# google/nerfactor

Measured on AMD Instinct MI355X. Metric: rays/sec (NeRF coarse+fine render, 64+128 samples/ray), higher is better.
Workload: dtype bf16; 1 GPU; lego_3072-shaped NeRF coarse+fine MLP render, 800x800 rays/view, 64+128 samples (BASELINE.json configs[1]); rays_per_view=640000, n_samples_coarse=64, n_samples_fine=128, kernel_variant=7

## Files before the change

include/nfx.h:

```cpp
#ifndef NFX_H_
#define NFX_H_

#include <stddef.h>
#include <stdint.h>

#ifdef __cplusplus
extern "C" {
#endif

#if defined(__GNUC__)
#define NFX_API __attribute__((visibility("default")))
#else
#define NFX_API
#endif

#define NFX_OK 0
#define NFX_EINVAL (-1)
#define NFX_EALIGN (-2)
#define NFX_EHIP (-3)
#define NFX_ENOSUP (-4)

#define NFX_PREC_BF16 0
#define NFX_PREC_FP32 1
#define NFX_PREC_FP32_NATIVE 2
// ... 236 lines not shown
                             void *dev_workspace, size_t workspace_bytes, void *stream);

NFX_API int nfx_nerf_refine_select(const float *dev_rgbs, const float *dev_z, const float *dev_rayd, int64_t n_rays,
                           int n_samples, float t_min, float a_lo, float a_hi, float sigma_margin, int dilate,
                           int *dev_list, int *dev_count, void *stream);
NFX_API int nfx_nerf_sigma_refine(const float *dev_rayo, const float *dev_rayd, const float *dev_z, int64_t n_rays,
                          int n_samples, const void *dev_geom_blob_fp32, const int *dev_list, const int *dev_count,
                          float *dev_rgbs, void *stream);

NFX_API int nfx_nerf_sigma_refine_last(const float *dev_rayo, const float *dev_rayd, const float *dev_z, int64_t n_rays,
                               int n_samples, const void *dev_geom_blob_fp32, float *dev_rgbs, void *stream);

#define NFX_OCCGRID_MAX_RES 1024
#define NFX_OCCGRID_MAX_PROBES (1ll << 30)
NFX_API int nfx_nerf_sigma_fwd_list(const float *dev_rayo, const float *dev_rayd, const float *dev_z, int64_t n_rays,
                            int n_samples, const void *dev_geom_blob, int prec, const int *dev_list,
                            const int *dev_count, float *dev_sigma, void *stream);
NFX_API size_t nfx_occgrid_workspace_bytes(int64_t n_rays, int n_samples);
NFX_API int nfx_occgrid_select(const float *dev_rayo, const float *dev_rayd, const float *dev_z, int64_t n_rays,
                       int n_samples, const uint32_t *dev_bits, int res, const float *box, const float *bbox,
                       float *dev_sigma, void *dev_workspace, size_t workspace_bytes, void *stream);
NFX_API int nfx_occgrid_bake(const float *dev_probe_sigma, int res, int probes, float margin, int dilate,
                     uint32_t *dev_bits, uint32_t *dev_workspace, void *stream);


NFX_API int nfx_selftest_mfma_bf16(const float *dev_a, const float *dev_b, float *dev_d, void *stream);
NFX_API int nfx_mlp_generic_split_hilo(void *dev_blob, int d_in, int n_layers, const int *widths, const int *skip_input,
                                       int train, void *stream);
NFX_API size_t nfx_mlp_generic_packed_bytes(int d_in, int n_layers, const int *widths, const int *skip_input, int prec);
NFX_API int nfx_mlp_generic_pack(const float *const *kernels, const float *const *biases, int d_in, int n_layers,
                                 const int *widths, const int *skip_input, int prec, void *blob, size_t blob_bytes);
NFX_API int nfx_mlp_generic_fwd(const float *dev_x, int64_t n, int ld_x, int d_in, int n_layers, const int *widths,
                                const int *acts, const int *skip_input, const void *dev_blob, int prec, float *dev_y,
                                int ld_y, int col0, void *stream);
NFX_API size_t nfx_mlp_generic_train_packed_bytes(int d_in, int n_layers, const int *widths, const int *skip_input,
                                                  int prec);
NFX_API int nfx_mlp_generic_pack_train(const float *const *kernels, const float *const *biases, int d_in, int n_layers,
                                       const int *widths, const int *skip_input, int prec, void *blob,
                                       size_t blob_bytes);
NFX_API size_t nfx_mlp_generic_bwd_workspace_bytes(int64_t n, int d_in, int n_layers, const int *widths,
                                                   const int *skip_input, int prec);
NFX_API int nfx_mlp_generic_bwd(const float *dev_x, int64_t n, int ld_x, int d_in, int n_layers, const int *widths,
                                const int *acts, const int *skip_input, const void *dev_train_blob, int prec,
                                const float *dev_dy, int ld_dy, int col0_dy, float *dev_dx, int ld_dx,
                                float *const *dev_dkernels, float *const *dev_dbiases, void *dev_workspace,
                                size_t workspace_bytes, void *stream);
NFX_API int nfx_embed_bwd(const float *dev_v, int64_t n, int n_freqs, int incl_input, const float *dev_d_out, int ld_out,
                          int col0, float *dev_dv, void *stream);
NFX_API int nfx_embed(const float *dev_x, const float *dev_dir, const float *dev_z, int64_t n, int per_ray, int mode,
                      int n_freqs, int incl_input, float *dev_out, int ld_out, int col0, void *stream);

NFX_API int nfx_selftest_tr16(const float *dev_h, const float *dev_z, float *dev_d, int mode, void *stream);
NFX_API int nfx_selftest_sincos(const float *dev_in, int64_t n, int which, float *dev_out, void *stream);

NFX_API int nfx_selftest_wgrad_plan(int n_calls, const int *k_in, const int *n_out, int64_t rows, int *use_lds, int *wide,
                                    int64_t *slab, int *n_slabs);
NFX_API size_t nfx_selftest_wgrad_partial_bytes(int n_calls, const int *k_in, const int *n_out, int64_t rows);
NFX_API int nfx_selftest_wgrad_batch(int n_calls, const void *const *dev_xt, const void *const *dev_zt, const int *k_in,
                                     const int *n_out, float *const *dev_dw, float *const *dev_db, int64_t ld, int64_t rows,
                                     const int32_t *dev_count, void *dev_partial, size_t partial_bytes, void *stream);

#ifdef __cplusplus
}
#endif
#endif
```

nerfactor_amd/_capi.py:

```python
import ctypes
import os

import torch

_HERE = os.path.dirname(os.path.abspath(__file__))
LIB_PATH = os.path.join(_HERE, 'libnfx.so')
if os.environ.get('NFX_LIB_PATH'):
    LIB_PATH = os.environ['NFX_LIB_PATH']

PREC_BF16, PREC_FP32, PREC_FP32_NATIVE = 0, 1, 2
ACT_NONE, ACT_RELU, ACT_SIGMOID, ACT_SOFTPLUS = 0, 1, 2, 3
IN_XYZ, IN_XYZ_LDIR, IN_Z_RUSINK = 0, 1, 2

if not os.path.exists(LIB_PATH):
    raise ImportError(
        "%s not found: build it with `python -m nerfactor_amd.build` (or __graft_entry__.build()); "
        "nerfactor_amd has no fallback path." % LIB_PATH)

lib = ctypes.CDLL(LIB_PATH)

_p = ctypes.c_void_p
_i = ctypes.c_int
_i64 = ctypes.c_int64
_f = ctypes.c_float
# ... 33 lines not shown
    'nfx_merl_query': (_i, [_p, _p, _i64, _p, _p, _p]),
    'nfx_merl_sphere_fwd': (_i, [_p, _p, _i64, _p, _p, _p, _p, _i, _p, _p, _p]),
    'nfx_dir2rusink': (_i, [_p, _p, _i64, _p, _p]),
    'nfx_mlp128_train_packed_bytes': (_sz, [_i]),
    'nfx_mlp128_pack_train_weights': (_i, [_pp, _pp, _i, _i, _i, _p, _sz]),
    'nfx_mlp128_bwd_workspace_bytes': (_sz, [_i, _i64, _i]),
    'nfx_mlp128_bwd': (_i, [_i, _p, _p, _i64, _f, _p, _i, _p, _i, _i, _f, _p, _p, _sz, _pp, _pp, _i, _p]),
    'nfx_mlp128_bwd_heads': (_i, [_i, _p, _p, _i64, _f, _p, _i, _i, _pp, _p, _p, _p, _pp, _p, _sz, _pp, _pp, _i, _p]),
    'nfx_composite_bwd': (_i, [_p, _p, _p, _p, _i64, _i, _i, _p, _p, _p]),
    'nfx_nerf_train_packed_bytes': (_sz, [_i]),
    'nfx_nerf_pack_train_weights': (_i, [_pp, _pp, _i, _p, _sz]),
    'nfx_nerf_bwd_workspace_bytes': (_sz, [_i64, _i]),
    'nfx_nerf_mlp_bwd': (_i, [_p, _p, _p, _i64, _i, _p, _i, _p, _p, _sz, _pp, _pp, _p]),
    'nfx_brdf_train_packed_bytes': (_sz, []),
    'nfx_brdf_pack_train_weights': (_i, [_pp, _pp, _i, _i, _p, _sz]),
    'nfx_brdf_spec_bwd_workspace_bytes': (_sz, [_i, _i64]),
    'nfx_brdf_spec_bwd': (_i, [_p, _p, _p, _p, _i, _p, _i, _p, _i, _i64, _p, _p, _p, _p, _sz, _p]),
    'nfx_brdf_spec_bwd_list_bytes': (_sz, [_i64, _i]),
    'nfx_brdf_spec_bwd_rows': (_i, [_p, _p, _p, _p, _i, _p, _i, _p, _i, _i64, _p, _p, _p, _p, _sz, _p, _sz, _p]),
    'nfx_brdf_rows_fwd': (_i, [_p, _i, _p, _i64, _i, _p, _i, _p, _p]),
    'nfx_brdf_rows_bwd_workspace_bytes': (_sz, [_i, _i64, _i]),
    'nfx_brdf_rows_bwd': (_i, [_p, _i, _p, _i64, _i, _p, _i, _p, _p, _sz, _p, _pp, _pp, _p]),
    'nfx_shade_bwd_workspace_bytes': (_sz, [_i]),
    'nfx_shade_bwd': (_i, [_p, _p, _p, _p, _p, _p, _f, _f, _p, _p, _p, _p, _i64, _i, _i, _p, _p, _p, _p, _p, _p,
                           _p, _p, _sz, _p]),
    'nfx_l2_normalize_rows': (_i, [_p, _p, _i64, _i, _f, _p]),
    'nfx_l2_normalize_rows_bwd': (_i, [_p, _p, _p, _i64, _i, _f, _p]),
    'nfx_light_smoothness': (_i, [_p, _i, _i, _f, _f, _p, _p, _p]),
    'nfx_pair_loss_fwd': (_i, [_p, _i, _p, _f, _i64, _p, _p]),
    'nfx_pair_loss_bwd': (_i, [_p, _i, _p, _f, _i64, _p, _p]),
    'nfx_pack_gather': (_i, [_p, _p, _i64, _p, _p]),
    'nfx_amsgrad_step': (_i, [_p, _p, _p, _p, _p, _i64, _f, _f, _f, _f, _i64, _p]),
    'nfx_amsgrad_step_size': (_f, [_f, _f, _f, _i64]),
    'nfx_amsgrad_step_dev': (_i, [_p, _p, _p, _p, _p, _i64, _p, _f, _f, _f, _p]),
    'nfx_nerf_sigma_fwd': (_i, [_p, _p, _p, _i64, _i, _p, _i, _p, _p]),
    'nfx_lvis_fwd_rows': (_i, [_p, _p, _i64, _f, _p, _i, _p, _i, _p, _sz, _p, _p, _p, _p]),
    'nfx_zero_rows': (_i, [_p, _p, _i64, _i, _p]),
    'nfx_shade_fwd_rows': (_i, [_p, _p, _p, _p, _p, _p, _f, _f, _p, _p, _p, _p, _p, _i64, _i, _i, _i, _p, _p]),
    'nfx_shade_olat_fwd_rows': (_i, [_p, _p, _p, _p, _p, _p, _f, _f, _p, _p, _p, _p, _f, _f, _i64, _i, _i, _p, _p, _p, _p]),
    'nfx_nerf_refine_select': (_i, [_p, _p, _p, _i64, _i, _f, _f, _f, _f, _i, _p, _p, _p]),
    'nfx_nerf_sigma_refine': (_i, [_p, _p, _p, _i64, _i, _p, _p, _p, _p, _p]),
    'nfx_nerf_sigma_refine_last': (_i, [_p, _p, _p, _i64, _i, _p, _p, _p]),
    'nfx_nerf_sigma_fwd_list': (_i, [_p, _p, _p, _i64, _i, _p, _i, _p, _p, _p, _p]),
    'nfx_occgrid_workspace_bytes': (_sz, [_i64, _i]),
    'nfx_occgrid_select': (_i, [_p, _p, _p, _i64, _i, _p, _i, _p, _p, _p, _p, _sz, _p]),
    'nfx_occgrid_bake': (_i, [_p, _i, _i, _f, _i, _p, _p, _p]),
    'nfx_nerf_geom_packed_bytes': (_sz, [_i]),
    'nfx_nerf_pack_geom_weights': (_i, [_pp, _pp, _i, _p, _sz]),
    'nfx_nerf_sigma_grad': (_i, [_p, _p, _p, _i64, _i, _p, _i, _p, _p]),
    'nfx_nerf_sigma_grad_workspace_bytes': (_sz, [_i64, _i]),
    'nfx_nerf_sigma_grad_rows': (_i, [_p, _p, _p, _i64, _i, _p, _i, _p, _p, _sz, _p]),
    'nfx_selftest_mfma_bf16': (_i, [_p, _p, _p, _p]),
    'nfx_selftest_sincos': (_i, [_p, _i64, _i, _p, _p]),
    'nfx_selftest_tr16': (_i, [_p, _p, _p, _i, _p]),
    'nfx_selftest_wgrad_plan': (_i, [_i, _p, _p, _i64, _p, _p, _p, _p]),
    'nfx_selftest_wgrad_partial_bytes': (_sz, [_i, _p, _p, _i64]),
    'nfx_selftest_wgrad_batch': (_i, [_i, _pp, _pp, _p, _p, _pp, _pp, _i64, _i64, _p, _p, _sz, _p]),
    'nfx_mlp_generic_packed_bytes': (_sz, [_i, _i, _p, _p, _i]),
    'nfx_mlp_generic_pack': (_i, [_pp, _pp, _i, _i, _p, _p, _i, _p, _sz]),
    'nfx_mlp_generic_fwd': (_i, [_p, _i64, _i, _i, _i, _p, _p, _p, _p, _i, _p, _i, _i, _p]),
    'nfx_mlp_generic_train_packed_bytes': (_sz, [_i, _i, _p, _p, _i]),
    'nfx_mlp_generic_pack_train': (_i, [_pp, _pp, _i, _i, _p, _p, _i, _p, _sz]),
    'nfx_mlp_generic_bwd_workspace_bytes': (_sz, [_i64, _i, _i, _p, _p, _i]),
    'nfx_mlp_generic_split_hilo': (_i, [_p, _i, _i, _p, _p, _i, _p]),
    'nfx_brdf_rows_geom_fwd': (_i, [_p, _p, _p, _p, _i, _p, _i, _i64, _i, _p, _i, _p, _p]),
    'nfx_brdf_rows_geom_bwd': (_i, [_p, _p, _p, _i, _p, _i, _i64, _i, _p, _i, _p, _p, _p]),
    'nfx_embed_bwd': (_i, [_p, _i64, _i, _i, _p, _i, _i, _p, _p]),
    'nfx_mlp_generic_bwd': (_i, [_p, _i64, _i, _i, _i, _p, _p, _p, _p, _i, _p, _i, _i, _p, _i, _pp, _pp, _p, _sz, _p]),
    'nfx_embed': (_i, [_p, _p, _p, _i64, _i, _i, _i, _i, _p, _i, _i, _p]),
}

for _name, (_res, _args) in SIGNATURES.items():
    _fn = getattr(lib, _name)
    _fn.restype = _res
    _fn.argtypes = _args


class NfxError(RuntimeError):
    """Raised for any non-zero return of the C-ABI; mirrors how the reference surfaces failures as
    Python exceptions (tf.errors.InvalidArgumentError from tf.debugging.*)."""


def last_error():
    buf = ctypes.create_string_buffer(512)
    lib.nfx_last_error(buf, 512)
    return buf.value.decode()


def check(rc, what):
    if rc != 0:
        raise NfxError("%s failed (%d): %s" % (what, rc, last_error()))


OPTION_KEYS = ('nerf_variant', 'nerf_fold', 'nerf_blocks', 'm128_blocks', 'lvis_variant', 'brdf_variant', 'brdf_ct', 'nerf_bwd',
               'nerf_bwd_nw', 'm128_bwd', 'wgrad_lds', 'wgrad_slabs', 'wgrad_rounds', 'wgrad_narrow', 'wgrad_fused', 'lvis_verify', 'lvis_rows', 'brdf_bwd_rows', 'nerf_bwd_rows', 'sigma_grad_rows', 'sigma_variant',
               'sigma_x3_variant')


def set_option(key, value):
    check(lib.nfx_set_option(key.encode(), int(value)), 'nfx_set_option(%s)' % key)


def unset_option(key):
    check(lib.nfx_unset_option(key.encode()), 'nfx_unset_option(%s)' % key)


# ... 32 lines not shown
```

nerfactor_amd/csrc/capi.cpp:

```cpp
#include <hip/hip_runtime.h>
#include <stdarg.h>
#include <stdio.h>
#include <stdlib.h>
#include <string.h>

#include <atomic>
#include <vector>

#include "capi_common.hpp"
#include "nerf_layout.hpp"
#include "nerf_fold_layout.hpp"
#include "pack.hpp"

static thread_local char g_err[512] = "";

int nfx_fail(int code, const char* fmt, ...) {
    va_list ap;
    va_start(ap, fmt);
    vsnprintf(g_err, sizeof(g_err), fmt, ap);
    va_end(ap);
    return code;
}
int nfx_hip_result(int e, const char* what) {
    if (e == 0) return NFX_OK;
// ... 244 lines not shown
int nfx_composite_fwd(const float* rgbs, const float* z, const float* rayd, const float* noise,
                      int64_t n_rays, int n_samples, int white_bg, float* rgb, float* occu, float* depth,
                      float* disp, float* weights, void* stream) {
    REQUIRE(n_rays >= 0 && n_samples >= 1, "nfx_composite_fwd: bad shape");
    if (n_rays == 0) return NFX_OK;
    REQUIRE(rgbs && z && rayd, "nfx_composite_fwd: null input");
    if (!ALIGNED(rgbs, 16)) return nfx_fail(NFX_EALIGN, "nfx_composite_fwd: rgbs must be 16-byte aligned");
    return nfx_hip_result(nfx_launch_composite(rgbs, z, rayd, noise, n_rays, n_samples, white_bg, rgb, occu,
                                               depth, disp, weights, (hipStream_t)stream),
                          "composite_fwd");
}

int nfx_nerf_surface_fwd(const float* sigma, const float* z, const float* rayo, const float* rayd, int64_t n_rays,
                         int n_samples, float occu_thres, int quantize_alpha, float* alpha, float* xyz, float* depth,
                         float* occu, void* stream) {
    REQUIRE(n_rays >= 0 && n_samples >= 1, "nfx_nerf_surface_fwd: bad shape (%lld rays, %d samples)", (long long)n_rays,
            n_samples);
    REQUIRE(occu_thres == occu_thres, "nfx_nerf_surface_fwd: occu_thres is NaN");
    if (n_rays == 0) return NFX_OK;
    REQUIRE(sigma && z && rayo && rayd, "nfx_nerf_surface_fwd: null input");
    REQUIRE(alpha && xyz && depth, "nfx_nerf_surface_fwd: null output (only occu may be NULL)");
    return nfx_hip_result(nfx_launch_surface(sigma, z, rayo, rayd, n_rays, n_samples, occu_thres, quantize_alpha ? 1 : 0, alpha,
                                             xyz, depth, occu, (hipStream_t)stream),
                          "nerf_surface_fwd");
}

int nfx_sample_fine(const float* z, const float* weights, int64_t n_rays, int n_coarse, int n_fine,
                    const float* u, float* z_all, void* stream) {
    REQUIRE(n_rays >= 0, "nfx_sample_fine: n_rays < 0");
    REQUIRE(n_coarse <= 258, "nfx_sample_fine: at most 258 coarse samples (256 pdf bins), got %d", n_coarse);
    REQUIRE(n_coarse >= 3 && n_fine >= 2, "nfx_sample_fine: need n_coarse >= 3 and n_fine >= 2 (got %d, %d)",
            n_coarse, n_fine);
    REQUIRE((size_t)4 * (2 * (n_coarse - 1) + n_coarse + n_fine) * 4 <= 64 * 1024,
            "nfx_sample_fine: n_coarse + n_fine too large for one workgroup's LDS");
    if (n_rays == 0) return NFX_OK;
    REQUIRE(z && weights && z_all, "nfx_sample_fine: null pointer");
    return nfx_hip_result(
            nfx_launch_sample_fine(z, weights, n_rays, n_coarse, n_fine, u, z_all, (hipStream_t)stream),
            "sample_fine");
}

int nfx_selftest_mfma_bf16(const float* a, const float* b, float* d, void* stream) {
    REQUIRE(a && b && d, "nfx_selftest_mfma_bf16: null pointer");
    return nfx_hip_result(nfx_launch_selftest_mfma(a, b, d, (hipStream_t)stream), "selftest_mfma");
}
int nfx_selftest_tr16(const float* h, const float* z, float* d, int mode, void* stream) {
    REQUIRE(d && (mode == 1 || (h && z)), "nfx_selftest_tr16: null pointer");
    return nfx_hip_result(nfx_launch_selftest_tr16(h, z, d, mode, (hipStream_t)stream), "selftest_tr16");
}
int nfx_selftest_sincos(const float* in, int64_t n, int which, float* out, void* stream) {
    REQUIRE(n >= 0 && (n == 0 || (in && out)), "nfx_selftest_sincos: bad arguments");
    return nfx_hip_result(nfx_launch_selftest_sincos(in, n, which, out, (hipStream_t)stream), "selftest_sincos");
}

}
```

nerfactor_amd/csrc/launchers.hpp:

```cpp
#pragma once
#include <hip/hip_runtime.h>
#include <stddef.h>
#include <stdint.h>

#include "../../include/nfx.h"

namespace nfx::generic { struct Args; struct EmbedArgs; struct BwdArgs; struct WgradArgs; }
namespace nfx::rowsgeom { struct Args; }
namespace nfx::geo { struct Points; }

struct nfx_wgrad_call {
    const void* xt;
    const void* zt;
    int k_in, n_out;
    float* dw;
    float* db;
};

extern "C" {
int nfx_option_int(const char* key, int dflt);
int nfx_brdf_train_blob_bytes(void);
int nfx_launch_brdf_spec_bwd(const float* xyz, const float* cam, const float* normal, const float* z, int z_dim, const float* lxyz,
                             int n_lights, const void* blob, long long n, const float* dspec, float* d_z, float* d_normal, void* workspace,
                             int max_blocks, hipStream_t st, void* list_ws);
// ... 48 lines not shown
int nfx_launch_split_hilo(void* frags, long long n_frags, hipStream_t st);
int nfx_launch_embed_bwd(const nfx::generic::EmbedArgs* a, const float* d_out, float* dv, hipStream_t st);
int nfx_launch_embed(const nfx::generic::EmbedArgs* a, hipStream_t st);
size_t nfx_nerf_bwd_list_bytes(long long n_pts);
int nfx_launch_nerf_bwd(const float* rayo, const float* rayd, const float* z, long long n_pts, int n_samples, const void* blob,
                        const float* d_rgbs, void* wsp, long long ld, int max_blocks, hipStream_t st, void* list_ws);
int nfx_launch_nerf_fold(const void* blob, void* out, hipStream_t stream);
int nfx_launch_nerf_sigma_grad(const nfx::geo::Points* pts, const void* blob, float* out, int max_blocks, hipStream_t st);
int nfx_launch_select_density(const float* sigma, long long n_pts, float* out, void* list_ws, hipStream_t st);
int nfx_launch_nerf_sigma_geo(const float* rayo, const float* rayd, const float* z, long long n_pts, int n_samples, const void* blob,
                              float* out, int max_blocks, hipStream_t st);
int nfx_launch_nerf_sigma_grad_x3(const nfx::geo::Points* pts, const void* blob, float* out, int max_blocks, hipStream_t st);
int nfx_launch_nerf_sigma_x3(const nfx::geo::Points* pts, const void* blob, float* out, int max_blocks, hipStream_t st);
int nfx_launch_nerf_mlp_bf16(const float* rayo, const float* rayd, const float* z, long long n_pts, int n_samples, const void* blob,
                             float* out, int variant, int max_blocks, hipStream_t stream);
int nfx_launch_nerf_mlp_bf16_fold(const float* rayo, const float* rayd, const float* z, long long n_pts, int n_samples, const void* blob,
                                  float* out, int variant, int max_blocks, hipStream_t stream);
int nfx_launch_nerf_mlp_bf16_v6(const float* rayo, const float* rayd, const float* z, long long n_pts, int n_samples, const void* blob,
                                float* out, int max_blocks, int dma_mode, hipStream_t stream);
int nfx_launch_nerf_mlp_bf16_v6_fold(const float* rayo, const float* rayd, const float* z, long long n_pts, int n_samples, const void* blob,
                                     float* out, int max_blocks, int dma_mode, hipStream_t stream);
int nfx_launch_nerf_mlp_x3(const float* rayo, const float* rayd, const float* z, long long n_pts, int n_samples, const void* blob,
                           float* out, int max_blocks, hipStream_t stream);
int nfx_launch_nerf_sigma_v6(const float* rayo, const float* rayd, const float* z, long long n_pts, int n_samples, const void* blob,
                             float* out, int max_blocks, hipStream_t stream);
int nfx_launch_nerf_sigma_v6_list(const float* rayo, const float* rayd, const float* z, long long capacity, int n_samples, const void* blob,
                                  float* out, const int* list, const int* count, int max_blocks, hipStream_t stream);
int nfx_launch_nerf_sigma_x3_pipe(const nfx::geo::Points* pts, const void* blob, float* out, int max_blocks, hipStream_t st);
size_t nfx_occgrid_list_bytes(long long n_pts);
int nfx_launch_occgrid_select(const float* rayo, const float* rayd, const float* z, long long n_rays, int n_samples, const uint32_t* bits,
                              int res, const float* box, const float* bbox, float* out, void* ws, hipStream_t st);
int nfx_launch_occgrid_bake(const float* sigma, int res, int probes, float margin, int dilate, uint32_t* bits, uint32_t* ws,
                            hipStream_t st);
int nfx_launch_pack_gather(const float* src, const int* map, long long n_words, void* blob, hipStream_t st);
int nfx_launch_l2_normalize3(const float* in, float* out, long long n, float eps, hipStream_t st);
int nfx_launch_gen_z(float near, float far, int n_samples, long long n_rays, int lin_in_disp, const float* u, float* z, hipStream_t st);
int nfx_launch_composite(const float* rgbs, const float* z, const float* rayd, const float* noise, long long n_rays, int S, int white_bg,
                         float* rgb, float* occu, float* depth, float* disp, float* w, hipStream_t st);
int nfx_launch_surface(const float* sigma, const float* z, const float* rayo, const float* rayd, long long n_rays, int S, float occu_thres,
                       int quantize, float* alpha, float* xyz, float* depth, float* occu, hipStream_t st);
int nfx_launch_refine_select(const float* rgbs, const float* z, const float* rayd, long long n_rays, int S, float t_min, float a_lo,
                             float a_hi, float sigma_margin, int dilate, int* list, int* count, hipStream_t st);
int nfx_launch_sample_fine(const float* z, const float* w, long long n_rays, int nc, int nf, const float* u, float* z_all, hipStream_t st);
int nfx_launch_composite_bwd(const float* rgbs, const float* z, const float* rayd, const float* noise, long long n_rays, int n_samples,
                             int white_bg, const float* d_rgb, float* d_rgbs, hipStream_t st);
int nfx_launch_scatter_rows(const float* src, const int* row_of, long long n_all, int d, float* dst, hipStream_t st);
int nfx_launch_zero_rows(float* dst, const int* row_of, long long n_all, int d, hipStream_t st);
int nfx_launch_nonfinite(const float* x, long long n, int* flag, hipStream_t st);
int nfx_launch_l2_normalize_rows(int bwd, const float* x, const float* dy, float* out, long long n, int d, float eps, hipStream_t st);
int nfx_launch_light_smoothness(const float* light, int H, int W, float tv_w, float achro_w, float* loss, float* grad, hipStream_t st);
int nfx_launch_selftest_tr16(const float* h, const float* z, float* d, int mode, hipStream_t st);
int nfx_launch_selftest_mfma(const float* a, const float* b, float* d, hipStream_t st);
int nfx_launch_selftest_sincos(const float* in, long long n, int which, float* out, hipStream_t st);
size_t nfx_shade_olat_lds_bytes(int n_lights);
int nfx_launch_shade(const float* xyz, const float* cam, const float* normal, const float* albedo, const float* rough, const float* spec,
                     float spec_scale, float f0, const float* lvis, const float* lxyz, const float* lareas, const float* lights,
                     long long n, int n_lights, int n_probes, int to_srgb, float* out, hipStream_t st, const int* lvis_row);
int nfx_launch_shade_olat(const float* xyz, const float* cam, const float* normal, const float* albedo, const float* rough,
                          const float* spec, float spec_scale, float f0, const float* lvis, const float* lxyz, const float* lareas,
                          float olat_inten, float ambient, long long n, int n_lights, int to_srgb, float* out, hipStream_t st,
                          const int* lvis_row, const int* out_row, int* nan_flag);
int nfx_launch_dir2rusink(const float* a, const float* b, long long n, float* out, hipStream_t st);
size_t nfx_shade_bwd_lds_bytes(int n_lights, int with_light_grad);
int nfx_launch_shade_bwd(const float* xyz, const float* cam, const float* normal, const float* albedo, const float* rough,
                         const float* spec, float spec_scale, float f0, const float* lvis, const float* lxyz, const float* lareas,
                         const float* light, long long n, int n_lights, int to_srgb, const float* drgb, float* d_albedo, float* d_rough,
                         float* d_spec, float* d_normal, float* d_lvis, float* d_light, void* workspace, hipStream_t st);
int nfx_launch_amsgrad(float* p, const float* g, float* m, float* v, float* vhat, long long n, float lr_t, float b1, float b2, float eps,
                       hipStream_t st);
int nfx_launch_amsgrad_dev(float* p, const float* g, float* m, float* v, float* vhat, long long n, const float* lr_t_dev, float b1,
                           float b2, float eps, hipStream_t st);
size_t nfx_wgrad_partial_bytes(const nfx_wgrad_call* calls, int n_calls, long long rows);
int nfx_launch_wgrad_batch_counted(const nfx_wgrad_call* calls, int n_calls, long long ld, long long rows, void* partial, const int* count,
                                   hipStream_t st);
int nfx_launch_wgrad_batch(const nfx_wgrad_call* calls, int n_calls, long long ld, long long rows, void* partial, hipStream_t st);
void nfx_wgrad_plan_of(const nfx_wgrad_call* calls, int n_calls, long long rows, int* form, long long* slab, int* n_slabs);
int nfx_wgrad_max_calls(void);
int nfx_wgrad_counted_ok(long long rows);
}
```

nerfactor_amd/csrc/mlp_engine.hpp:

```cpp
#pragma once
#include <type_traits>
#include "nfx_common.hpp"

namespace nfx {

constexpr int kFragBytes = 1024;
constexpr int kSlotFrags = 24;
constexpr int kSlotBytes = kSlotFrags * kFragBytes;
constexpr int kPieceThreads = 256;


template <int B, int E, typename F>
__device__ __forceinline__ void static_for(F&& f) {
    if constexpr (B < E) {
        f(std::integral_constant<int, B>{});
        static_for<B + 1, E>(f);
    }
}

struct WStream {
    const u32x4* gnext;
    const u32x4* gbase;
    const u32x4* gend;
    char* ring;
// ... 191 lines not shown
          int KS2A, int NTA, int CT>
__device__ __forceinline__ void layer_pre(WStream& ws, int tid, const float* __restrict__ pre,
                                          const bf16x8 (&b1)[KS1A][CT],
                                          const bf16x8 (&b2)[KS2A][CT], bf16x8 (&bout)[NTA][CT]) {
    static_assert(2 * NT <= NTA, "output array too small");
    const int h = (tid & 63) >> 5;
    static_for<0, NT>([&](auto T) {
        constexpr int t = decltype(T)::value;
        f32x16 acc[CT];
        tile_init<KS1, KS2, (t == NT - 1 ? NL_NEXT : NL_SELF), NW>(
            ws, tid, [&](f32x16(&a)[CT]) { vec_init<CT>(pre + 32 * t, h, a); }, b1, b2, acc);
        acc_to_b<RELU, CT>(acc, bout[2 * t], bout[2 * t + 1]);
    });
}

template <int L>
struct PeSlots {
    static constexpr int kKS = (3 * L + 2 + 7) / 8;
};

template <int L, int CT>
__device__ __forceinline__ void posenc(const float (&x)[3], int h, int c,
                                       bf16x8 (&out)[PeSlots<L>::kKS][CT]) {
    constexpr int NQ = PeSlots<L>::kKS * 8;
    float v[NQ];
#pragma unroll
    for (int q = 3 * L; q < NQ; ++q) v[q] = q == 3 * L ? (h ? x[2] : x[0]) : (q == 3 * L + 1 && !h) ? x[1] : 0.0f;
    if constexpr (L <= 4) {
#pragma unroll
        for (int q = 0; q < 3 * L; ++q) v[q] = sin_shifted_small(x[q % 3] * (float)(1 << (q / 3)), h);
    } else {
#pragma unroll
        for (int d = 0; d < 3; ++d)
#pragma unroll
            for (int k0 = 0; k0 < L; k0 += 5) {
                float sn, cs;
                sincos_cw(x[d] * (float)(1 << k0), sn, cs);
#pragma unroll
                for (int k = k0; k < k0 + 5 && k < L; ++k) {
                    v[3 * k + d] = h ? cs : sn;
                    const float s2 = 2.0f * sn * cs;
                    cs = fmaf(-2.0f * sn, sn, 1.0f);
                    sn = s2;
                }
            }
    }
#pragma unroll
    for (int s = 0; s < PeSlots<L>::kKS; ++s) {
#pragma unroll
        for (int j = 0; j < 8; ++j) out[s][c][j] = (__bf16)v[8 * s + j];
    }
}

}
```

nerfactor_amd/csrc/nerf_mlp_v6.hip:

```cpp
#include "nerf_v6_engine.hpp"
#include "launchers.hpp"

namespace nfx {
namespace v6 {

template <int DMA, Seq S>
__device__ __forceinline__ void nerf_mlp_bf16_v6_body(
    const float* __restrict__ rayo, const float* __restrict__ rayd, const float* __restrict__ zbuf, long long n_pts,
    int n_samples, const char* __restrict__ blob, float4* __restrict__ out) {
    extern __shared__ __attribute__((aligned(16))) char smem[];
    using namespace nerf;
    const int tid = threadIdx.x, lane = tid & 63, wave = tid >> 6, h = lane >> 5, p = lane & 31;
    constexpr bool FOLD = S == Seq::Render;
    float* bias_lds = floats_of<DMA, S>(smem);
    Acc accs[2];
    Pre pre;
    Regs rg;
    const Ctx cx = prologue<DMA, S>(smem, blob, FOLD ? nerf::fold::kWeightBytes : nerf::kWeightBytes, kBiasFloats, tid, lane, rg, pre,
                                    accs[0]);
    const long long n_tiles = (n_pts + kTilePts - 1) / kTilePts;
    for (long long tl = blockIdx.x; tl < n_tiles; tl += gridDim.x) {
        bf16x8 pe[4][kCT], pv[2][kCT];
        long long m[kCT];
#pragma unroll
        for (int c = 0; c < kCT; ++c) {
            m[c] = tl * kTilePts + wave * (32 * kCT) + c * 32 + p;
            const long long mm = m[c] < n_pts ? m[c] : n_pts - 1;
            const long long ray = mm / n_samples;
            const float zz = zbuf[mm];
            float x[3], d[3];
#pragma unroll
            for (int k = 0; k < 3; ++k) {
                d[k] = rayd[ray * 3 + k];
                x[k] = rayo[ray * 3 + k] + d[k] * zz;
            }
            posenc<10, kCT>(x, h, c, pe);
            posenc<4, kCT>(d, h, c, pv);
        }
        bf16x8 ha[16][kCT], hb[16][kCT], r0[8][kCT];
        float sigma[kCT];
        const float* bl = bias_lds + kBiasL0;
        auto pend = [&](auto relu_tag, const Acc& a, bf16x8(&lo)[kCT], bf16x8(&hi)[kCT]) {
            return EpiB<decltype(relu_tag)::value>{a, lo, hi};
        };
        using T = std::true_type;
        using F = std::false_type;
        layer<0, 4, 0, 8, true, DMA, S>(cx, rg, bl, bl + 256 * 1, pe, pe, ha, accs, pre, EpiNone{});
        layer<8, 16, 0, 8, true, DMA, S>(cx, rg, bl + 256 * 1, bl + 256 * 2, ha, pe, hb, accs, pre, pend(T{}, accs[1], ha[14], ha[15]));
        layer<16, 16, 0, 8, true, DMA, S>(cx, rg, bl + 256 * 2, bl + 256 * 3, hb, pe, ha, accs, pre, pend(T{}, accs[1], hb[14], hb[15]));
        layer<24, 16, 0, 8, true, DMA, S>(cx, rg, bl + 256 * 3, bl + 256 * 4, ha, pe, hb, accs, pre, pend(T{}, accs[1], ha[14], ha[15]));
        layer<32, 16, 0, 8, true, DMA, S>(cx, rg, bl + 256 * 4, bl + 256 * 5, hb, pe, ha, accs, pre, pend(T{}, accs[1], hb[14], hb[15]));
        layer<40, 16, 4, 8, true, DMA, S>(cx, rg, bl + 256 * 5, bl + 256 * 6, ha, pe, hb, accs, pre, pend(T{}, accs[1], ha[14], ha[15]));
        layer<48, 16, 0, 8, true, DMA, S>(cx, rg, bl + 256 * 6, bl + 256 * 7, hb, pe, ha, accs, pre, pend(T{}, accs[1], hb[14], hb[15]));
        if constexpr (FOLD) {
        layer<56, 16, 0, 8, true, DMA, S>(cx, rg, bl + 256 * 7, bias_lds + kBiasBott + 256, ha, pe, hb, accs, pre, pend(T{}, accs[1], ha[14], ha[15]));
        tile<64, 16, 0, DMA, S>(cx, rg, bias_lds + kBiasRgb0, hb, pe, accs[0], accs[1], pre, pend(T{}, accs[1], hb[14], hb[15]));
        {
            EpiSigma es{accs[0], sigma};
            layer<65, 16, 2, 4, true, DMA, S>(cx, rg, bias_lds + kBiasRgb0, bias_lds + kBiasRgb1, hb, pv, r0, accs, pre, es);
        }
        tile<69, 8, 0, DMA, S>(cx, rg, bl, r0, pe, accs[1], accs[0], pre, pend(T{}, accs[0], r0[6], r0[7]));
        } else {
        layer<56, 16, 0, 8, true, DMA, S>(cx, rg, bl + 256 * 7, bias_lds + kBiasBott, ha, pe, hb, accs, pre, pend(T{}, accs[1], ha[14], ha[15]));
        layer<64, 16, 0, 8, false, DMA, S>(cx, rg, bias_lds + kBiasBott, bias_lds + kBiasBott + 256, hb, pe, ha, accs, pre,
                                       pend(T{}, accs[1], hb[14], hb[15]));
        tile<72, 16, 0, DMA, S>(cx, rg, bias_lds + kBiasRgb0, hb, pe, accs[0], accs[1], pre, pend(F{}, accs[1], ha[14], ha[15]));
        {
            EpiSigma es{accs[0], sigma};
            layer<73, 16, 2, 4, true, DMA, S>(cx, rg, bias_lds + kBiasRgb0, bias_lds + kBiasRgb1, ha, pv, r0, accs, pre, es);
        }
        tile<77, 8, 0, DMA, S>(cx, rg, bl, r0, pe, accs[1], accs[0], pre, pend(T{}, accs[0], r0[6], r0[7]));
        }
        if (h == 0) {
#pragma unroll
            for (int c = 0; c < kCT; ++c)
                if (m[c] < n_pts) out[m[c]] = make_float4(accs[1].v[c][0], accs[1].v[c][1], accs[1].v[c][2], sigma[c]);
        }
    }
}

template <int AB, int DMA>
__global__ __launch_bounds__(kNW * 64, 1) void nerf_mlp_bf16_v6_kernel(
    const float* __restrict__ rayo, const float* __restrict__ rayd, const float* __restrict__ zbuf, long long n_pts,
    int n_samples, const char* __restrict__ blob, float4* __restrict__ out) {
    nerf_mlp_bf16_v6_body<DMA, Seq::Packed>(rayo, rayd, zbuf, n_pts, n_samples, blob, out);
}

namespace fold {
template <int AB, int DMA>
__global__ __launch_bounds__(kNW * 64, 1) void nerf_mlp_bf16_v6_kernel(
// ... 36 lines not shown
```

nerfactor_amd/csrc/selftest.hip:

```cpp
#include "nfx_common.hpp"
#include "tr16.hpp"
#include "launchers.hpp"

namespace nfx {
__global__ void selftest_mfma_kernel(const float* A, const float* B, float* D) {
    const int l = threadIdx.x, h = l >> 5, n = l & 31;
    bf16x8 a, b;
#pragma unroll
    for (int j = 0; j < 8; ++j) {
        a[j] = (__bf16)A[n * 16 + 8 * h + j];
        b[j] = (__bf16)B[(8 * h + j) * 32 + n];
    }
    f32x16 acc;
#pragma unroll
    for (int r = 0; r < 16; ++r) acc[r] = 0.f;
    acc = __builtin_amdgcn_mfma_f32_32x32x16_bf16(a, b, acc, 0, 0, 0);
#pragma unroll
    for (int r = 0; r < 16; ++r) D[((r & 3) + 8 * (r >> 2) + 4 * h) * 32 + n] = acc[r];
}
__global__ void selftest_sincos_kernel(const float* in, long long n, int which, float* out) {
    const long long i = (long long)blockIdx.x * blockDim.x + threadIdx.x;
    if (i < n) out[i] = which < 2 ? sin_shifted(in[i], which) : sin_shifted_small(in[i], which - 2);
}
__global__ void selftest_tr16_kernel(const float* H, const float* Z, float* D, int mode) {
    __shared__ __attribute__((aligned(16))) char lds[2 * 16 * 288];
    constexpr int P = 288;
    const int l = threadIdx.x;
    if (mode == 1) {
        short* e = reinterpret_cast<short*>(lds);
        for (int i = l; i < 1024; i += 64) e[i] = (short)i;
        __syncthreads();
        const s16x4 v = __builtin_amdgcn_ds_read_tr16_b64_v4i16((lds_s16x4*)(lds + 8 * l));
        for (int j = 0; j < 4; ++j) D[l * 4 + j] = (float)v[j];
        return;
    }
    for (int i = l; i < 16 * 32; i += 64) {
        const int row = i >> 5, slot = i & 31;
        *reinterpret_cast<__bf16*>(lds + row * P + slot * 2) = (__bf16)H[i];
        *reinterpret_cast<__bf16*>(lds + 16 * P + row * P + slot * 2) = (__bf16)Z[i];
    }
    __syncthreads();
    const int off = tr_lane_off(l, P);
    const bf16x8 a = tr_frag<P>(lds + off), b = tr_frag<P>(lds + 16 * P + off);
    f32x16 acc;
#pragma unroll
    for (int r = 0; r < 16; ++r) acc[r] = 0.f;
    acc = __builtin_amdgcn_mfma_f32_32x32x16_bf16(a, b, acc, 0, 0, 0);
#pragma unroll
    for (int r = 0; r < 16; ++r) D[((r & 3) + 8 * (r >> 2) + 4 * (l >> 5)) * 32 + (l & 31)] = acc[r];
}
}

extern "C" {
int nfx_launch_selftest_tr16(const float* h, const float* z, float* d, int mode, hipStream_t st) {
    hipLaunchKernelGGL(nfx::selftest_tr16_kernel, dim3(1), dim3(64), 0, st, h, z, d, mode);
    return (int)hipGetLastError();
}
int nfx_launch_selftest_mfma(const float* a, const float* b, float* d, hipStream_t st) {
    hipLaunchKernelGGL(nfx::selftest_mfma_kernel, dim3(1), dim3(64), 0, st, a, b, d);
    return (int)hipGetLastError();
}
int nfx_launch_selftest_sincos(const float* in, long long n, int which, float* out, hipStream_t st) {
    if (n <= 0) return 0;
    hipLaunchKernelGGL(nfx::selftest_sincos_kernel, dim3((unsigned)((n + 255) / 256)), dim3(256), 0, st,
                       in, n, which, out);
    return (int)hipGetLastError();
}
}
```

nerfactor_amd/ops.py:

```python
import ctypes
import os

import numpy as np
import torch

from . import _capi
from ._capi import PREC_BF16, PREC_FP32, PREC_FP32_NATIVE, check, lib

_PREC = {'bf16': PREC_BF16, 'fp32': PREC_FP32, 'fp32_native': PREC_FP32_NATIVE, PREC_BF16: PREC_BF16, PREC_FP32: PREC_FP32,
         PREC_FP32_NATIVE: PREC_FP32_NATIVE}
_ACT = {None: 0, 'none': 0, 'relu': 1, 'sigmoid': 2, 'softplus': 3}


def _ptr(t):
    return None if t is None else ctypes.c_void_p(t.data_ptr())


def _stream():
    return ctypes.c_void_p(torch.cuda.current_stream().cuda_stream)


def _dev(t, name, shape=None):
    if t is None:
        return None
# ... 434 lines not shown
    x = _dev(x, 'x', (None, 3))
    if not isinstance(d_out, torch.Tensor) or not d_out.is_cuda or d_out.dtype != torch.float32 or d_out.dim() != 2 \
            or d_out.stride(1) != 1 or d_out.shape[0] != x.shape[0]:
        raise _capi.NfxError("embed_bwd: d_out must be a CUDA fp32 matrix with one row per vector")
    dx = torch.empty_like(x)
    check(lib.nfx_embed_bwd(_ptr(x), x.shape[0], n_freqs, int(incl_input), _ptr(d_out), d_out.stride(0) if x.shape[0] else 0,
                            col0, _ptr(dx), _stream()), 'nfx_embed_bwd')
    return dx


def embed(n_freqs, incl_input=True, x=None, rayo=None, rayd=None, z=None, per_ray=1, out=None, col0=0, lights=None):
    d_out = (3 if incl_input else 0) + 6 * n_freqs
    if lights is not None:
        mode, a, b, c = 3, _dev(x, 'x', (None, 3)), _dev(lights, 'lights', (None, 3)), None
        per_ray = b.shape[0]
        n = a.shape[0] * per_ray
    elif z is not None:
        mode, n, per_ray = 1, z.numel(), z.shape[1]
        a, b, c = _dev(rayo, 'rayo', (None, 3)), _dev(rayd, 'rayd', (None, 3)), _dev(z, 'z')
    elif x is not None:
        mode, a, b, c = 0, _dev(x, 'x', (None, 3)), None, None
        n = a.shape[0] * per_ray
    else:
        mode, a, b, c = 2, None, _dev(rayd, 'rayd', (None, 3)), None
        n = b.shape[0] * per_ray
    dev_ = (a if a is not None else b).device
    if out is None:
        out = torch.empty((n, col0 + d_out), dtype=torch.float32, device=dev_)
    _check_out('embed', out, n, col0, d_out, dev_)
    check(lib.nfx_embed(_ptr(a), _ptr(b), _ptr(c), n, per_ray, mode, n_freqs, 1 if incl_input else 0, _ptr(out),
                        out.stride(0) if n else d_out, col0, _stream()), 'nfx_embed')
    return out


def selftest_tr16(h=None, z=None):
    if h is None:
        d = torch.empty((64, 4), dtype=torch.float32, device='cuda')
        check(lib.nfx_selftest_tr16(None, None, _ptr(d), 1, _stream()), 'nfx_selftest_tr16')
        return d
    h, z = _dev(h, 'h', (16, 32)), _dev(z, 'z', (16, 32))
    d = torch.empty((32, 32), dtype=torch.float32, device=h.device)
    check(lib.nfx_selftest_tr16(_ptr(h), _ptr(z), _ptr(d), 0, _stream()), 'nfx_selftest_tr16')
    return d


def selftest_sincos(x, which):
    x = _dev(x, 'x')
    out = torch.empty_like(x)
    check(lib.nfx_selftest_sincos(_ptr(x), x.numel(), int(which), _ptr(out), _stream()),
          'nfx_selftest_sincos')
    return out


def _wgrad_dims(dims):
    n = len(dims)
    return n, (ctypes.c_int * n)(*[int(d[0]) for d in dims]), (ctypes.c_int * n)(*[int(d[1]) for d in dims])


def selftest_wgrad_plan(dims, rows):
    n, k, o = _wgrad_dims(dims)
    use_lds, wide, n_slabs, slab = ctypes.c_int(0), ctypes.c_int(0), ctypes.c_int(0), ctypes.c_int64(0)
    check(lib.nfx_selftest_wgrad_plan(n, k, o, int(rows), ctypes.byref(use_lds), ctypes.byref(wide), ctypes.byref(slab),
                                      ctypes.byref(n_slabs)), 'nfx_selftest_wgrad_plan')
    return {'use_lds': bool(use_lds.value), 'wide': bool(wide.value), 'slab': slab.value, 'n_slabs': n_slabs.value}


def selftest_wgrad_partial_bytes(dims, rows):
    n, k, o = _wgrad_dims(dims)
    return int(lib.nfx_selftest_wgrad_partial_bytes(n, k, o, int(rows)))


def selftest_wgrad_batch(calls, ld, rows, partial, count=None, partial_bytes=None):
    n, k, o = _wgrad_dims([(c[2], c[3]) for c in calls])
    col = lambda j: (ctypes.c_void_p * n)(*[None if c[j] is None else c[j].data_ptr() for c in calls])
    if partial_bytes is None:
        partial_bytes = partial.numel() * partial.element_size()
    check(lib.nfx_selftest_wgrad_batch(n, col(0), col(1), k, o, col(4), col(5), int(ld), int(rows), _ptr(count), _ptr(partial),
                                       int(partial_bytes), _stream()), 'nfx_selftest_wgrad_batch')


def mlp128_xyz_fwd(xyz, blob, out_dim, out_act=None, xyz_scale=1., post_scale=1., post_bias=0.,
                   prec='bf16'):
    xyz = _dev(xyz, 'xyz', (None, 3))
    n = xyz.shape[0]
    out = torch.empty((n, out_dim), dtype=torch.float32, device=xyz.device)
    check(lib.nfx_mlp128_xyz_fwd(_ptr(xyz), n, xyz_scale, _ptr(blob), out_dim, _ACT[out_act],
                                 post_scale, post_bias, _PREC[prec], _ptr(out), _stream()),
          'nfx_mlp128_xyz_fwd')
    return out


def lvis_rows_supported(prec='bf16'):
    return prec == 'bf16' and _capi.get_option("lvis_variant") in (None, 8, 2, 3, 4) and _capi.get_option("lvis_rows") == 1


def zero_rows(dst, row_of):
    dst = _dev(dst, 'dst', (row_of.shape[0], None))
    if not row_of.is_cuda or row_of.dtype != torch.int32 or not row_of.is_contiguous():
        raise _capi.NfxError("zero_rows: row_of must be a contiguous CUDA int32 tensor")
    check(lib.nfx_zero_rows(_ptr(dst), ctypes.c_void_p(row_of.data_ptr()), dst.shape[0], dst.shape[1], _stream()), 'nfx_zero_rows')
    return dst


def lvis_fwd(xyz, lxyz, blob, xyz_scale=1., xyz_dir=None, prec='bf16', out=None, out_row=None, nan_flag=None):
    xyz = _dev(xyz, 'xyz', (None, 3))
    xyz_dir = _dev(xyz_dir, 'xyz_dir', (xyz.shape[0], 3))
# ... 645 lines not shown
```

Before: 5.316 million rays/s.

## Split posenc10 across half-waves with permlane swap and incremental ray indexing

```diff
diff --git a/include/nfx.h b/include/nfx.h
--- a/include/nfx.h
+++ b/include/nfx.h
@@ -312,6 +312,7 @@
 
 NFX_API int nfx_selftest_tr16(const float *dev_h, const float *dev_z, float *dev_d, int mode, void *stream);
 NFX_API int nfx_selftest_sincos(const float *dev_in, int64_t n, int which, float *dev_out, void *stream);
+NFX_API int nfx_selftest_posenc10(const float *dev_x, int64_t n, int split, float *dev_out, void *stream);
 
 NFX_API int nfx_selftest_wgrad_plan(int n_calls, const int *k_in, const int *n_out, int64_t rows, int *use_lds, int *wide,
                                     int64_t *slab, int *n_slabs);
diff --git a/nerfactor_amd/_capi.py b/nerfactor_amd/_capi.py
--- a/nerfactor_amd/_capi.py
+++ b/nerfactor_amd/_capi.py
@@ -109,6 +109,7 @@
     'nfx_nerf_sigma_grad_rows': (_i, [_p, _p, _p, _i64, _i, _p, _i, _p, _p, _sz, _p]),
     'nfx_selftest_mfma_bf16': (_i, [_p, _p, _p, _p]),
     'nfx_selftest_sincos': (_i, [_p, _i64, _i, _p, _p]),
+    'nfx_selftest_posenc10': (_i, [_p, _i64, _i, _p, _p]),
     'nfx_selftest_tr16': (_i, [_p, _p, _p, _i, _p]),
     'nfx_selftest_wgrad_plan': (_i, [_i, _p, _p, _i64, _p, _p, _p, _p]),
     'nfx_selftest_wgrad_partial_bytes': (_sz, [_i, _p, _p, _i64]),
diff --git a/nerfactor_amd/csrc/capi.cpp b/nerfactor_amd/csrc/capi.cpp
--- a/nerfactor_amd/csrc/capi.cpp
+++ b/nerfactor_amd/csrc/capi.cpp
@@ -320,5 +320,9 @@
     REQUIRE(n >= 0 && (n == 0 || (in && out)), "nfx_selftest_sincos: bad arguments");
     return nfx_hip_result(nfx_launch_selftest_sincos(in, n, which, out, (hipStream_t)stream), "selftest_sincos");
 }
-
-}
+int nfx_selftest_posenc10(const float* x, int64_t n, int split, float* out, void* stream) {
+    REQUIRE(n >= 0 && (n == 0 || (x && out)), "nfx_selftest_posenc10: bad arguments");
+    return nfx_hip_result(nfx_launch_selftest_posenc10(x, n, split, out, (hipStream_t)stream), "selftest_posenc10");
+}
+
+}
diff --git a/nerfactor_amd/csrc/launchers.hpp b/nerfactor_amd/csrc/launchers.hpp
--- a/nerfactor_amd/csrc/launchers.hpp
+++ b/nerfactor_amd/csrc/launchers.hpp
@@ -124,6 +124,7 @@
 int nfx_launch_selftest_tr16(const float* h, const float* z, float* d, int mode, hipStream_t st);
 int nfx_launch_selftest_mfma(const float* a, const float* b, float* d, hipStream_t st);
 int nfx_launch_selftest_sincos(const float* in, long long n, int which, float* out, hipStream_t st);
+int nfx_launch_selftest_posenc10(const float* x, long long n, int split, float* out, hipStream_t st);
 size_t nfx_shade_olat_lds_bytes(int n_lights);
 int nfx_launch_shade(const float* xyz, const float* cam, const float* normal, const float* albedo, const float* rough, const float* spec,
                      float spec_scale, float f0, const float* lvis, const float* lxyz, const float* lareas, const float* lights,
diff --git a/nerfactor_amd/csrc/mlp_engine.hpp b/nerfactor_amd/csrc/mlp_engine.hpp
--- a/nerfactor_amd/csrc/mlp_engine.hpp
+++ b/nerfactor_amd/csrc/mlp_engine.hpp
@@ -267,4 +267,31 @@
     }
 }
 
-}
+template <int CT>
+__device__ __forceinline__ void posenc10_split(const float (&x)[3], int h, int c, bf16x8 (&out)[PeSlots<10>::kKS][CT]) {
+    constexpr int L = 10, NQ = PeSlots<L>::kKS * 8;
+    float v[NQ];
+#pragma unroll
+    for (int q = 3 * L; q < NQ; ++q) v[q] = q == 3 * L ? (h ? x[2] : x[0]) : (q == 3 * L + 1 && !h) ? x[1] : 0.0f;
+#pragma unroll
+    for (int d = 0; d < 3; ++d) {
+        float sn, cs;
+        sincos_cw(h ? x[d] * (float)(1 << 5) : x[d], sn, cs);
+#pragma unroll
+        for (int i = 0; i < 5; ++i) {
+            const auto sw = __builtin_amdgcn_permlane32_swap(__float_as_uint(sn), __float_as_uint(cs), false, false);
+            v[3 * i + d] = __uint_as_float(sw[0]);
+            v[3 * (i + 5) + d] = __uint_as_float(sw[1]);
+            const float s2 = 2.0f * sn * cs;
+            cs = fmaf(-2.0f * sn, sn, 1.0f);
+            sn = s2;
+        }
+    }
+#pragma unroll
+    for (int s = 0; s < PeSlots<L>::kKS; ++s) {
+#pragma unroll
+        for (int j = 0; j < 8; ++j) out[s][c][j] = (__bf16)v[8 * s + j];
+    }
+}
+
+}
diff --git a/nerfactor_amd/csrc/nerf_mlp_v6.hip b/nerfactor_amd/csrc/nerf_mlp_v6.hip
--- a/nerfactor_amd/csrc/nerf_mlp_v6.hip
+++ b/nerfactor_amd/csrc/nerf_mlp_v6.hip
@@ -19,23 +19,55 @@
     const Ctx cx = prologue<DMA, S>(smem, blob, FOLD ? nerf::fold::kWeightBytes : nerf::kWeightBytes, kBiasFloats, tid, lane, rg, pre,
                                     accs[0]);
     const long long n_tiles = (n_pts + kTilePts - 1) / kTilePts;
+    const bool idx32 = n_pts < (1ll << 31);
+    const unsigned ns = (unsigned)n_samples;
+    const unsigned qp = idx32 ? (unsigned)p / ns : 0u, rp = (unsigned)p - qp * ns;
+    const unsigned q32 = idx32 ? 32u / ns : 0u, r32 = 32u - q32 * ns;
+    const unsigned ray_last = idx32 ? (unsigned)(n_pts - 1) / ns : 0u;
+    const unsigned wave_pt = (unsigned)__builtin_amdgcn_readfirstlane(wave) * (32 * kCT);
     for (long long tl = blockIdx.x; tl < n_tiles; tl += gridDim.x) {
         bf16x8 pe[4][kCT], pv[2][kCT];
-        long long m[kCT];
+        long long m[kCT], rays[kCT];
+#pragma unroll
+        for (int c = 0; c < kCT; ++c) m[c] = tl * kTilePts + wave * (32 * kCT) + c * 32 + p;
+        if (idx32) {
+            const unsigned m0 = (unsigned)tl * kTilePts + wave_pt;
+            unsigned rc = m0 / ns, sc = m0 - rc * ns;
+#pragma unroll
+            for (int c = 0; c < kCT; ++c) {
+                const unsigned s = sc + rp;
+                const unsigned r = rc + qp + (s >= ns ? 1u : 0u);
+                rays[c] = r < ray_last ? r : ray_last;
+                sc += r32;
+                rc += q32 + (sc >= ns ? 1u : 0u);
+                sc -= sc >= ns ? ns : 0u;
+            }
+        } else {
+#pragma unroll
+            for (int c = 0; c < kCT; ++c) {
+                const long long mm = m[c] < n_pts ? m[c] : n_pts - 1;
+                const long long ray = mm / n_samples;
+                rays[c] = ray;
+            }
+        }
+        float zz[kCT], o[kCT][3], d[kCT][3];
 #pragma unroll
         for (int c = 0; c < kCT; ++c) {
-            m[c] = tl * kTilePts + wave * (32 * kCT) + c * 32 + p;
-            const long long mm = m[c] < n_pts ? m[c] : n_pts - 1;
-            const long long ray = mm / n_samples;
-            const float zz = zbuf[mm];
-            float x[3], d[3];
+            const long long ray = rays[c];
+            zz[c] = zbuf[m[c] < n_pts ? m[c] : n_pts - 1];
 #pragma unroll
             for (int k = 0; k < 3; ++k) {
-                d[k] = rayd[ray * 3 + k];
-                x[k] = rayo[ray * 3 + k] + d[k] * zz;
+                d[c][k] = rayd[ray * 3 + k];
+                o[c][k] = rayo[ray * 3 + k];
             }
-            posenc<10, kCT>(x, h, c, pe);
-            posenc<4, kCT>(d, h, c, pv);
+        }
+#pragma unroll
+        for (int c = 0; c < kCT; ++c) {
+            float x[3];
+#pragma unroll
+            for (int k = 0; k < 3; ++k) x[k] = o[c][k] + d[c][k] * zz[c];
+            posenc10_split<kCT>(x, h, c, pe);
+            posenc<4, kCT>(d[c], h, c, pv);
         }
         bf16x8 ha[16][kCT], hb[16][kCT], r0[8][kCT];
         float sigma[kCT];
diff --git a/nerfactor_amd/csrc/selftest.hip b/nerfactor_amd/csrc/selftest.hip
--- a/nerfactor_amd/csrc/selftest.hip
+++ b/nerfactor_amd/csrc/selftest.hip
@@ -1,5 +1,6 @@
 #include "nfx_common.hpp"
 #include "tr16.hpp"
+#include "mlp_engine.hpp"
 #include "launchers.hpp"
 
 namespace nfx {
@@ -21,6 +22,20 @@
 __global__ void selftest_sincos_kernel(const float* in, long long n, int which, float* out) {
     const long long i = (long long)blockIdx.x * blockDim.x + threadIdx.x;
     if (i < n) out[i] = which < 2 ? sin_shifted(in[i], which) : sin_shifted_small(in[i], which - 2);
+}
+__global__ void selftest_posenc10_kernel(const float* x, long long n, int split, float* out) {
+    const int l = threadIdx.x, h = l >> 5;
+    const long long i = (long long)blockIdx.x * 32 + (l & 31), ii = i < n ? i : n - 1;
+    const float xs[3] = {x[ii * 3], x[ii * 3 + 1], x[ii * 3 + 2]};
+    bf16x8 pe[4][1];
+    if (split) posenc10_split<1>(xs, h, 0, pe);
+    else posenc<10, 1>(xs, h, 0, pe);
+    if (i < n) {
+#pragma unroll
+        for (int s = 0; s < 4; ++s)
+#pragma unroll
+            for (int j = 0; j < 8; ++j) out[(i * 2 + h) * 32 + 8 * s + j] = (float)pe[s][0][j];
+    }
 }
 __global__ void selftest_tr16_kernel(const float* H, const float* Z, float* D, int mode) {
     __shared__ __attribute__((aligned(16))) char lds[2 * 16 * 288];
@@ -60,6 +75,11 @@
     hipLaunchKernelGGL(nfx::selftest_mfma_kernel, dim3(1), dim3(64), 0, st, a, b, d);
     return (int)hipGetLastError();
 }
+int nfx_launch_selftest_posenc10(const float* x, long long n, int split, float* out, hipStream_t st) {
+    if (n <= 0) return 0;
+    hipLaunchKernelGGL(nfx::selftest_posenc10_kernel, dim3((unsigned)((n + 31) / 32)), dim3(64), 0, st, x, n, split, out);
+    return (int)hipGetLastError();
+}
 int nfx_launch_selftest_sincos(const float* in, long long n, int which, float* out, hipStream_t st) {
     if (n <= 0) return 0;
     hipLaunchKernelGGL(nfx::selftest_sincos_kernel, dim3((unsigned)((n + 255) / 256)), dim3(256), 0, st,
diff --git a/nerfactor_amd/ops.py b/nerfactor_amd/ops.py
--- a/nerfactor_amd/ops.py
+++ b/nerfactor_amd/ops.py
@@ -510,6 +510,13 @@
     return out
 
 
+def selftest_posenc10(x, split):
+    x = _dev(x, 'x', (None, 3))
+    out = torch.empty((x.shape[0], 2, 32), dtype=torch.float32, device=x.device)
+    check(lib.nfx_selftest_posenc10(_ptr(x), x.shape[0], 1 if split else 0, _ptr(out), _stream()), 'nfx_selftest_posenc10')
+    return out
+
+
 def _wgrad_dims(dims):
     n = len(dims)
     return n, (ctypes.c_int * n)(*[int(d[0]) for d in dims]), (ctypes.c_int * n)(*[int(d[1]) for d in dims])
```

Result: no change. 5.363 million rays/s (median of 6 runs) (+0.9%).
